# NonStopEagle137/Visual-Inertial-Odometry-MSCKF-Stereo

Measured on AMD Instinct MI355X. Metric: EKF measurement updates/sec at 30 cam-states x 200 features; ATE RMSE vs ref, higher is better.
Workload: dtype f32/f64; 1 GPU; batched EKF measurement update, 30 cam-states x 200 features, 2048 filters/GPU, triangulation + jacobian + gating + information assembly + Kalman, no row cap; cam_states=30, features=200, filters_per_gpu=2048, parallelism=replicas1

## Files before the change

visual-inertial-odometry-msckf-stereo_amd/csrc/msckf_kalman.hip:

```cpp
#include "msckf_common.h"
#include "msckf_launch.h"
#include "msckf_mchol_slots.h"
#include "msckf_rchol.h"

#include <stdlib.h>
#include <type_traits>

namespace msckf {

constexpr int KW = 24;

__device__ __forceinline__ int round4(int x) { return (x + 3) & ~3; }


typedef double v4d __attribute__((ext_vector_type(4)));

constexpr double KALMAN_PIVOT_FLOOR = 1e-10;

template <typename T>
__device__ double diag_max(const T* M, int ld, int o, int n, double* lds) {
    double m = 0.0;
    for (int i = threadIdx.x; i < n; i += blockDim.x) m = fmax(m, (double)M[(size_t)(o + i) * (ld + 1)]);
    m = wave_max(m);
    if ((threadIdx.x & 63) == 0) lds[threadIdx.x >> 6] = m;
    __syncthreads();
    for (int w = 0; w < (int)(blockDim.x >> 6); ++w) m = fmax(m, lds[w]);
    __syncthreads();
    return m;
}
template <typename T>
__device__ double pcc_pivot_floor(const T* P, int ld, int C, double* lds) {
    return diag_max(P, ld, 21, C, lds) * KALMAN_PIVOT_FLOOR;
}
constexpr double T_FLOOR_NEG = 1e-9;

template <typename T, int NT, int TPL, bool RETRY = false>
__global__ void __launch_bounds__(NT) __attribute__((amdgpu_waves_per_eu(NT == 256 ? 2 : 1))) k_kal_a(DevState<T> st, UpdWs<T> ws) {
    extern __shared__ __attribute__((aligned(16))) unsigned char smem_raw[];
    const int b = blockIdx.x;
    if (RETRY && ws.afail[b] == 0) return;
    const int C = 6 * st.ncams[b], Cp = round4(C);
    const int nrow = (Cp + KW) / 4;
    const T* P = st.P + (size_t)b * st.Dmax * st.Dmax;
    const int ld = st.Dmax, Cpw = ws.Cp;
    KT* Lc = ws.Lc + (size_t)b * Cpw * Cpw;
    KT* Vi = ws.Vi + (size_t)b * KW * Cpw;
    KT* Sii = ws.Sii + (size_t)b * KW * KW;
    auto map = [&](int i) { return i < C ? 21 + i : (i < Cp ? -1 : (i < Cp + 21 ? i - Cp : -1)); };
    double shift = 0.0;
    auto load = [&](int i, int j) -> double {
        const int mi = map(i), mj = map(j);
        if (mi < 0 || mj < 0) return i == j ? 1.0 : 0.0;
        return (double)P[(size_t)mi * ld + mj] + (i == j && i < C ? shift : 0.0);
    };
    auto panel = [&](int r, int c0, double w0, double w1, double w2, double w3) {
        KT* dst = r < Cp ? Lc + (size_t)r * Cpw + c0 : Vi + (size_t)(r - Cp) * Cpw + c0;
        dst[0] = w0; dst[1] = w1; dst[2] = w2; dst[3] = w3;
    };
    auto trail = [&](int i, int j, double v) { Sii[(i - Cp) * KW + (j - Cp)] = v; };
    const double floor = pcc_pivot_floor(P, ld, C, reinterpret_cast<double*>(smem_raw));
    bool ok = false;
    for (int att = RETRY ? 1 : 0; att < (RETRY ? 3 : 1) && !ok; ++att) {
        if (att > 0) {
            shift = (att == 1 ? 1e-8 : 1e-6) * (floor / KALMAN_PIVOT_FLOOR);
            __syncthreads();
        }
        ok = rchol_core<NT, TPL>(nrow, nrow, Cp / 4, reinterpret_cast<double*>(smem_raw), load, panel, trail, floor);
    }
    if (threadIdx.x == 0) ws.afail[b] = ok ? 0 : 1;
}

template <typename T, int NT, int TPL>
__global__ void __launch_bounds__(NT) __attribute__((amdgpu_waves_per_eu(NT == 256 ? 2 : 1))) k_kal_c1(DevState<T> st, UpdWs<T> ws) {
    extern __shared__ __attribute__((aligned(16))) unsigned char smem_raw[];
    const int b = blockIdx.x;
    if (ws.info[4 * b] == 0) return;
    if (ws.afail[b]) {
        if (threadIdx.x == 0) ws.info[4 * b + 3] = -2;
        return;
    }
    const int C = 6 * st.ncams[b], Cp = round4(C), nTc = Cp / 4;
    const int ldt = ws.Cmax + 1;
    const KT* Tm = ws.Tm + (size_t)b * ws.Cmax * ldt;
    KT* L = ws.G + (size_t)b * ws.Cmax * ldt;
    const bool rev = ws.rev;
    auto load = [&](int i, int j) -> double {
        if (i >= C || j >= C) return i == j ? 1.0 : 0.0;
        const int ri = rev ? C - 1 - i : i, rj = rev ? C - 1 - j : j;
        return ri >= rj ? Tm[(size_t)ri * ldt + rj] : Tm[(size_t)rj * ldt + ri];
    };
    auto panel = [&](int r, int c0, double w0, double w1, double w2, double w3) {
        if (r >= C) return;
        KT* dst = L + (size_t)r * ldt;
        const double w[4] = {w0, w1, w2, w3};
#pragma unroll
        for (int q = 0; q < 4; ++q)
            if (c0 + q < C && c0 + q <= r) dst[c0 + q] = w[q];
    };
    auto trail = [](int, int, double) {};
    const double tmax = diag_max(Tm, ldt, 0, C, reinterpret_cast<double*>(smem_raw));
    const bool ok = rchol_core<NT, TPL>(nTc, nTc, nTc, reinterpret_cast<double*>(smem_raw), load, panel, trail, ws.s2,
                                        -T_FLOOR_NEG * tmax);
    if (!ok && threadIdx.x == 0) ws.info[4 * b + 3] = -1;
}

constexpr int C2S = 17;

template <typename T, int NW, int CT, int NTM>
__global__ void __launch_bounds__(64 * NW) k_kal_c2(DevState<T> st, UpdWs<T> ws) {
    extern __shared__ __attribute__((aligned(16))) unsigned char smem_raw[];
    constexpr int NT = 64 * NW;
    const int b = blockIdx.x;
    if (ws.info[4 * b] == 0 || ws.info[4 * b + 3] < 0) return;
    const int C = 6 * st.ncams[b], nT = (C + 15) / 16, E = 22 + C, nE = (E + 15) / 16;
    const int tid = threadIdx.x, lane = tid & 63, lc = lane & 15, lr = lane >> 4;
    const int wv = __builtin_amdgcn_readfirstlane(tid >> 6);
    const int ldt = ws.Cmax + 1, Cpw = ws.Cp, ldw = st.Dmax + 1;
    const KT* L = ws.G + (size_t)b * ws.Cmax * ldt;
    const KT* Tm = ws.Tm + (size_t)b * ws.Cmax * ldt;
    const KT* Lc = ws.Lc + (size_t)b * Cpw * Cpw;
    const KT* Vi = ws.Vi + (size_t)b * KW * Cpw;
    KT* Wt = ws.W + (size_t)b * (st.Dmax + 1) * Cpw;
    double* LI = reinterpret_cast<double*>(smem_raw);
    double* img = LI + NTM * 256;
    auto Lv = [&](int r, int k) -> double {
        if (r >= C || k >= C) return r == k ? 1.0 : 0.0;
        return k <= r ? L[(size_t)r * ldt + k] : 0.0;
    };
    for (int J = wv; J < nT; J += NW) {
        double* blk = img + wv * 272;
#pragma unroll
        for (int q = 0; q < 4; ++q) {
            const int e = lane + 64 * q, i = e >> 4, k = e & 15;
            blk[e] = Lv(16 * J + i, 16 * J + k);
        }
        __builtin_amdgcn_wave_barrier();
        __builtin_amdgcn_fence(__ATOMIC_ACQ_REL, "wavefront");
        if (lane < 16) blk[256 + lane] = 1.0 / blk[17 * lane];
        __builtin_amdgcn_wave_barrier();
        __builtin_amdgcn_fence(__ATOMIC_ACQ_REL, "wavefront");
        if (lane < 16) {
            double x[16];
#pragma unroll
            for (int i = 0; i < 16; ++i) {
                double sv = i == lane ? 1.0 : 0.0;
#pragma unroll
                for (int k = 0; k < i; ++k) sv -= k >= lane ? blk[16 * i + k] * x[k] : 0.0;
                x[i] = i < lane ? 0.0 : sv * blk[256 + i];
            }
            double* xj = LI + J * 256 + 16 * lane;
#pragma unroll
            for (int i = 0; i < 16; ++i) xj[i] = x[i];
        }
        __builtin_amdgcn_wave_barrier();
        __builtin_amdgcn_fence(__ATOMIC_ACQ_REL, "wavefront");
    }
    const bool rev = ws.rev;
    auto Xv = [&](int e, int k) -> double {
        if (k >= C) return 0.0;
        const int j = rev ? C - 1 - k : k;
        if (e < 21) return Vi[(size_t)e * Cpw + j];
        if (e < 21 + C) return j <= e - 21 ? Lc[(size_t)(e - 21) * Cpw + j] : 0.0;
        if (e == 21 + C) return Tm[(size_t)j * ldt + C];
        return 0.0;
    };
    v4d yk[CT][NTM];
    int J0[CT];
#pragma unroll
// ... 265 lines not shown
#pragma unroll
        for (int q = 0; q < NLD; ++q) {
            int ii, kk, jj, k2;
            idx(q, A_KFAST, ii, kk);
            idx(q, B_KFAST, jj, k2);
            const int gi = i0 + ii, gk = k0 + kk;
            ra[q] = (gi < m && gk < ke) ? A(gi, gk) : 0.0;
            const int gj = j0 + jj, gk2 = k0 + k2;
            rb[q] = (gj < n && gk2 < ke) ? B(gk2, gj) : 0.0;
        }
    };
    auto sstore = [&](int bf) {
#pragma unroll
        for (int q = 0; q < NLD; ++q) {
            int ii, kk, jj, k2;
            idx(q, A_KFAST, ii, kk);
            idx(q, B_KFAST, jj, k2);
            sa[bf][kk][ii] = ra[q];
            sb[bf][k2][jj] = rb[q];
        }
    };
    if (kb < ke) {
        gload(kb);
        sstore(0);
    }
    __syncthreads();
    for (int k0 = kb, it = 0; k0 < ke; k0 += GK, ++it) {
        const int bf = it & 1;
        const bool more = k0 + GK < ke;
        if (more) gload(k0 + GK);
#pragma unroll
        for (int kc = 0; kc < GK / 4; ++kc) {
            const int kr = 4 * kc + lr;
            double av[NBW], bv[NBW];
#pragma unroll
            for (int t = 0; t < NBW; ++t) {
                av[t] = sa[bf][kr][HW * wr + 16 * t + lc];
                bv[t] = sb[bf][kr][HW * wc + 16 * t + lc];
            }
#pragma unroll
            for (int mi = 0; mi < NBW; ++mi)
#pragma unroll
                for (int ni = 0; ni < NBW; ++ni)
                    acc[mi][ni] = __builtin_amdgcn_mfma_f64_16x16x4f64(av[mi], bv[ni], acc[mi][ni], 0, 0, 0);
        }
        if (more) sstore(bf ^ 1);
        __syncthreads();
    }
#pragma unroll
    for (int mi = 0; mi < NBW; ++mi)
#pragma unroll
        for (int ni = 0; ni < NBW; ++ni)
#pragma unroll
            for (int r = 0; r < 4; ++r) {
                const int i = i0 + HW * wr + 16 * mi + lr + 4 * r, j = j0 + HW * wc + 16 * ni + lc;
                if (i < m && j < n) store(i, j, acc[mi][ni][r]);
            }
}
template <bool A_KFAST, bool B_KFAST, class FA, class FB, class FS>
__device__ __forceinline__ void gemm64(int m, int n, int kb, int ke, int i0, int j0, FA A, FB B, FS store) {
    gemm_tile<64, A_KFAST, B_KFAST>(m, n, kb, ke, i0, j0, A, B, store);
}

template <int STAGE, typename T>
__global__ void __launch_bounds__(256) k_gchol_trsm(DevState<T> st, UpdWs<T> ws, int k) {
    const Blk3 bk = xcd_blk3();
    const int b = bk.y;
    KT* A;
    int nrow, ncol, nelim;
    if (!gdims<STAGE>(st, ws, b, A, nrow, ncol, nelim) || k >= nelim) return;
    const int ld = ncol, nb = nelim - k < GNB ? nelim - k : GNB;
    const int i0 = k + nb + bk.x * GT;
    if (i0 >= nrow) return;
    const KT* Li = ws.G + (size_t)b * ws.Cmax * (ws.Cmax + 1);
    gemm64<true, true>(nrow, nb, 0, nb, i0, 0,
                       [&](int i, int p) { return A[(size_t)i * ld + k + p]; },
                       [&](int p, int j) { return Li[j * GNB + p]; },
                       [&](int i, int j, double v) { A[(size_t)i * ld + k + j] = v; });
}

template <int STAGE, typename T>
__global__ void __launch_bounds__(256) k_gchol_update(DevState<T> st, UpdWs<T> ws, int k) {
    const Blk3 bk = xcd_blk3();
    const int b = bk.z;
    KT* A;
    int nrow, ncol, nelim;
    if (!gdims<STAGE>(st, ws, b, A, nrow, ncol, nelim) || k >= nelim) return;
    const int ld = ncol, k1 = k + (nelim - k < GNB ? nelim - k : GNB);
    const int i0 = k1 + bk.y * GT, j0 = k1 + bk.x * GT;
    if (i0 >= nrow || j0 >= ncol || i0 + GT - 1 < j0) return;
    gemm64<true, true>(nrow, ncol, k, k1, i0, j0,
                       [&](int i, int p) { return A[(size_t)i * ld + p]; },
                       [&](int p, int j) { return A[(size_t)j * ld + p]; },
                       [&](int i, int j, double v) {
                           if (j <= i) A[(size_t)i * ld + j] -= v;
                       });
}

template <typename T>
__global__ void __launch_bounds__(256) k_kal_b1(DevState<T> st, UpdWs<T> ws) {
    const Blk3 bk = xcd_blk3();
    const int b = bk.z;
    if (ws.info[4 * b] == 0) return;
    const int C = 6 * st.ncams[b];
    const int i0 = bk.y * GT, j0 = bk.x * GT;
    if (i0 >= C || j0 >= C) return;
    const int lda = ws.Cmax + 1, Cpw = ws.Cp;
    const KT* Am = ws.Hthin + (size_t)b * ws.Cmax * lda;
    const KT* Lc = ws.Lc + (size_t)b * Cpw * Cpw;
    KT* G = ws.G + (size_t)b * ws.Cmax * lda;
    gemm64<true, false>(C, C, j0 & ~(GK - 1), C, i0, j0,
                        [&](int i, int k) { return Am[(size_t)i * lda + k]; },
                        [&](int k, int j) { return k >= j ? Lc[(size_t)k * Cpw + j] : 0.0; },
                        [&](int i, int j, double v) { G[(size_t)i * lda + j] = v; });
}

template <typename T>
__global__ void __launch_bounds__(256) k_kal_b2(DevState<T> st, Params<T> prm, UpdWs<T> ws) {
    const Blk3 bk = xcd_blk3();
    const int b = bk.z;
    if (ws.info[4 * b] == 0) return;
    const int C = 6 * st.ncams[b];
    const int i0 = bk.y * GT, j0 = bk.x * GT;
    if (i0 >= C || j0 > C) return;
    if (j0 > i0 + GT - 1 && !(C >= j0 && C < j0 + GT)) return;
    const int ld = ws.Cmax + 1, Cpw = ws.Cp;
    const KT* Lc = ws.Lc + (size_t)b * Cpw * Cpw;
    const KT* G = ws.G + (size_t)b * ws.Cmax * ld;
    const KT* Hb = ws.Hthin + (size_t)b * ws.Cmax * ld;
    KT* Tm = ws.Tm + (size_t)b * ws.Cmax * ld;
    KT* Ac = ws.Wk + (size_t)b * ws.wk_stride + gchol_c_off(ws.Cmax);
    const double s2 = (double)prm.sigma2;
    gemm64<false, false>(C, C + 1, i0 & ~(GK - 1), C, i0, j0,
                         [&](int i, int k) { return k >= i ? Lc[(size_t)k * Cpw + i] : 0.0; },
                         [&](int k, int j) { return j < C ? G[(size_t)k * ld + j] : Hb[(size_t)k * ld + ws.Cmax]; },
                         [&](int i, int j, double v) {
                             if (j < C && j <= i) {
                                 const double t = v + (i == j ? s2 : 0.0);
                                 Ac[(size_t)i * C + j] = t;
                                 if (i == j) Tm[(size_t)i * ld + i] = t;
                             }
                             if (j == C) Ac[(size_t)(2 * C + 21) * C + i] = v;
                         });
}

__device__ __forceinline__ void lower_tile(int t, int& ti, int& tj) {
    int i = (int)((sqrtf(8.0f * (float)t + 1.0f) - 1.0f) * 0.5f);
    while (i * (i + 1) / 2 > t) --i;
    while ((i + 1) * (i + 2) / 2 <= t) ++i;
    ti = i;
    tj = t - i * (i + 1) / 2;
}

template <typename T, int NW, int NTM>
__global__ void __launch_bounds__(64 * NW) k_kal_b(DevState<T> st, Params<T> prm, UpdWs<T> ws) {
    constexpr int TP2 = (NTM * (NTM + 1) / 2 + NW - 1) / NW;
    constexpr int NT = 64 * NW, Q = (16 * 16 * NTM + NT - 1) / NT;
    extern __shared__ __attribute__((aligned(16))) unsigned char smem_raw[];
    const int b = blockIdx.x;
    if (ws.info[4 * b] == 0) return;
    const int C = 6 * st.ncams[b], nT = (C + 15) / 16, Cq = 16 * nT;
    const int tid = threadIdx.x, lane = tid & 63, lc = lane & 15, lr = lane >> 4;
    const int wv = __builtin_amdgcn_readfirstlane(tid >> 6);
    const int ld = ws.Cmax + 1, Cpw = ws.Cp;
    const KT* Am = ws.Hthin + (size_t)b * ws.Cmax * ld;
    const KT* Lc = ws.Lc + (size_t)b * Cpw * Cpw;
    KT* G = ws.G + (size_t)b * ws.Cmax * ld;
    KT* Tm = ws.Tm + (size_t)b * ws.Cmax * ld;
    const int CqS1 = (Cq & ~31) + 17, CqS2 = (Cq & ~31) + 16;
    double* img = reinterpret_cast<double*>(smem_raw);
    double* bb = img + 4 * 16 * CqS1;
    double r0[Q], r1[Q], rb = 0.0;
    int pos[Q];
    auto load = [&](int ph, int k0) {
#pragma unroll
        for (int q = 0; q < Q; ++q) {
            const int e = tid + NT * q;
            int k, c;
            if (ph == 0) {
                const int jt = e >> 8, u = e & 255;
                const bool up = jt > (k0 >> 4);
                k = up ? (u & 15) : (u >> 4);
                c = 16 * jt + (up ? (u >> 4) : (u & 15));
            } else {
                k = e / Cq;
                c = e - k * Cq;
            }
            const int gk = k0 + k;
            pos[q] = k * (ph == 0 ? CqS1 : CqS2) + c;
            const bool in = e < 16 * Cq && gk < C && c < C;
            const double lcv = (in && c <= gk) ? Lc[(size_t)gk * Cpw + c] : 0.0;
            double ov;
            if (ph == 0) {
                ov = in ? Am[c <= gk ? (size_t)gk * ld + c : (size_t)c * ld + gk] : 0.0;
            } else {
                ov = (in && c < 16 * (gk / 16 + 1)) ? G[(size_t)gk * ld + c] : 0.0;
            }
            r0[q] = ph == 0 ? ov : lcv;
            r1[q] = ph == 0 ? lcv : ov;
        }
        if (ph == 1 && tid < 16) rb = k0 + tid < C ? Am[(size_t)(k0 + tid) * ld + ws.Cmax] : 0.0;
    };
    auto put = [&](int ph, int buf) {
        const int CqS = ph == 0 ? CqS1 : CqS2;
        double* i0 = img + (2 * buf) * 16 * CqS;
#pragma unroll
        for (int q = 0; q < Q; ++q) {
            const int e = tid + NT * q;
            if (e < 16 * Cq) {
                i0[pos[q]] = r0[q];
                i0[16 * CqS + pos[q]] = r1[q];
            }
        }
        if (ph == 1 && tid < 16) bb[buf * 16 + tid] = rb;
    };
    {
        const int CqS = CqS1;
        const int ntl = nT * (nT + 1) / 2;
        v4d acc[TP2];
        int gr[TP2], gc[TP2];
#pragma unroll
        for (int s = 0; s < TP2; ++s) {
            const int t = wv + NW * s, tt = t < ntl ? t : 0;
            const int c = colmajor_col(tt, nT), r = c + tt - (c * nT - c * (c - 1) / 2);
            gr[s] = __builtin_amdgcn_readfirstlane(t < ntl ? r : -1);
            gc[s] = __builtin_amdgcn_readfirstlane(c);
            acc[s] = v4d{0.0, 0.0, 0.0, 0.0};
        }
        load(0, 0);
        put(0, 0);
        __syncthreads();
        for (int k0 = 0, it = 0; k0 < C; k0 += 16, ++it) {
            const int buf = it & 1;
            const bool more = k0 + 16 < C;
            if (more) load(0, k0 + 16);
            const double* i0 = img + (2 * buf) * 16 * CqS;
            const double* i1 = i0 + 16 * CqS;
#pragma unroll
            for (int kc = 0; kc < 4; ++kc) {
                const int kr = (4 * kc + lr) * CqS;
#pragma unroll
                for (int s = 0; s < TP2; ++s) {
                    if (gr[s] < 0 || k0 + 15 < 16 * gc[s]) continue;
                    acc[s] = __builtin_amdgcn_mfma_f64_16x16x4f64(i0[kr + 16 * gr[s] + lc], i1[kr + 16 * gc[s] + lc],
                                                                  acc[s], 0, 0, 0);
                }
            }
            if (more) put(0, buf ^ 1);
            __syncthreads();
        }
#pragma unroll
        for (int s = 0; s < TP2; ++s) {
            if (gr[s] < 0) continue;
#pragma unroll
            for (int r = 0; r < 4; ++r) {
                const int i = 16 * gr[s] + lr + 4 * r, j = 16 * gc[s] + lc;
                if (i < C && j < C) G[(size_t)i * ld + j] = acc[s][r];
            }
        }
        __syncthreads();
    }
    {
        const int CqS = CqS2;
        const int ntl = nT * (nT + 1) / 2;
        v4d acc[TP2];
        int ti[TP2], tj[TP2];
#pragma unroll
        for (int s = 0; s < TP2; ++s) {
            const int t = wv + NW * s;
            int x, y;
            lower_tile(t, x, y);
            ti[s] = __builtin_amdgcn_readfirstlane(t < ntl ? x : -1);
            tj[s] = __builtin_amdgcn_readfirstlane(y);
            acc[s] = v4d{0.0, 0.0, 0.0, 0.0};
        }
        double ca = 0.0;
        load(1, 0);
        put(1, 0);
        __syncthreads();
        for (int k0 = 0, it = 0; k0 < C; k0 += 16, ++it) {
            const int buf = it & 1;
            const bool more = k0 + 16 < C;
            if (more) load(1, k0 + 16);
            const double* i0 = img + (2 * buf) * 16 * CqS;
            const double* i1 = i0 + 16 * CqS;
#pragma unroll
            for (int kc = 0; kc < 4; ++kc) {
                const int kr = (4 * kc + lr) * CqS;
#pragma unroll
                for (int s = 0; s < TP2; ++s) {
                    if (ti[s] < 0 || k0 + 15 < 16 * ti[s]) continue;
                    acc[s] = __builtin_amdgcn_mfma_f64_16x16x4f64(i0[kr + 16 * ti[s] + lc], i1[kr + 16 * tj[s] + lc],
                                                                  acc[s], 0, 0, 0);
                }
            }
            if (tid < C) {
#pragma unroll
                for (int k = 0; k < 16; ++k) ca += i0[k * CqS + tid] * bb[buf * 16 + k];
            }
            if (more) put(1, buf ^ 1);
            __syncthreads();
        }
        const double s2 = (double)prm.sigma2;
#pragma unroll
        for (int s = 0; s < TP2; ++s) {
            if (ti[s] < 0) continue;
#pragma unroll
            for (int r = 0; r < 4; ++r) {
                const int i = 16 * ti[s] + lr + 4 * r, j = 16 * tj[s] + lc;
                if (i < C && j <= i) Tm[(size_t)i * ld + j] = acc[s][r] + (i == j ? s2 : 0.0);
            }
        }
        if (tid < C) Tm[(size_t)tid * ld + C] = ca;
    }
}

template <typename T>
__global__ void __launch_bounds__(256) __attribute__((amdgpu_waves_per_eu(2))) k_kal_e(DevState<T> st, Params<T> prm, UpdWs<T> ws) {
    constexpr int TE = 128;
    const Blk3 bk = xcd_blk3();
    const int b = bk.z;
    if (ws.info[4 * b] == 0 || ws.info[4 * b + 3] < 0) return;
    const int C = 6 * st.ncams[b], D = 21 + C;
    const int i0 = bk.y * TE, j0 = bk.x * TE;
    if (i0 >= D || j0 > D) return;
    if (j0 > i0 + TE - 1 && !(D >= j0 && D < j0 + TE)) return;
    const int ld = st.Dmax;
    const KT* W = ws.Wk + (size_t)b * ws.wk_stride + gchol_c_off(ws.Cmax) + (size_t)C * C;
    const KT* Sii = ws.Sii + (size_t)b * KW * KW;
    T* P = st.P + (size_t)b * st.Dmax * st.Dmax;
    KT* dx = ws.dx + (size_t)b * (st.Dmax + ws.Cmax);
    const double s2 = (double)prm.sigma2;
    gemm_tile<TE, true, true>(D, D + 1, 0, C, i0, j0, [&](int i, int k) { return W[(size_t)i * C + k]; },
                       [&](int k, int j) { return W[(size_t)(j < D ? j : D) * C + k]; },
                       [&](int i, int j, double v) {
                           if (j < D && j <= i) {
                               double p = s2 * v;
                               if (i < 21 && j < 21) p += Sii[i * KW + j];
                               P[(size_t)i * ld + j] = (T)p;
                               P[(size_t)j * ld + i] = (T)p;
                           }
                           if (j == D) dx[i] = v;
                       });
}

template <typename T, int NW, int TPW>
__global__ void __launch_bounds__(64 * NW) k_kal_e1(DevState<T> st, Params<T> prm, UpdWs<T> ws) {
    extern __shared__ __attribute__((aligned(16))) unsigned char smem_raw[];
    const int b = blockIdx.x;
    if (ws.info[4 * b] == 0 || ws.info[4 * b + 3] < 0) return;
    const int C = 6 * st.ncams[b], D = 21 + C, nT = (D + 15) / 16, Dp = 16 * nT;
    const int tid = threadIdx.x, lane = tid & 63, lc = lane & 15, lr = lane >> 4;
    const int wv = __builtin_amdgcn_readfirstlane(tid >> 6);
    const int ntiles = nT * (nT + 1) / 2;
    const int Cpw = ws.Cp, ld = st.Dmax;
    const KT* W = ws.W + (size_t)b * (st.Dmax + 1) * Cpw;
    double* img = reinterpret_cast<double*>(smem_raw);
    double* yb = img + 2 * 16 * Dp;
    int ti[TPW], tj[TPW], kf[TPW];
#pragma unroll
    for (int s = 0; s < TPW; ++s) {
        const int t = wv + NW * s;
        int c = 0, rem = t;
        if (rem >= nT) {
            rem -= nT;
            c = 1;
            if (rem >= nT - 1) {
                rem -= nT - 1;
                c = nT - 1;
                while (c > 1 && rem >= nT - c) { rem -= nT - c; --c; }
            }
        }
        const int rmax = (16 * c + 15 < D ? 16 * c + 15 : D - 1) - 21;
        ti[s] = __builtin_amdgcn_readfirstlane(t < ntiles ? c + rem : -1);
        tj[s] = __builtin_amdgcn_readfirstlane(c);
        kf[s] = __builtin_amdgcn_readfirstlane(ws.rev && c >= 2 ? (C - 1 - rmax) / 16 : 0);
    }
    v4d acc[TPW];
#pragma unroll
    for (int s = 0; s < TPW; ++s) acc[s] = v4d{0.0, 0.0, 0.0, 0.0};
    double dxa = 0.0, dxb = 0.0;
    constexpr int NT = 64 * NW, Q = (16 * 16 * (NW * TPW <= 96 ? 13 : 15) + NT - 1) / NT;
    double rw[Q], ry = 0.0;
    const int ldw = st.Dmax + 1;
    auto load = [&](int k0) {
#pragma unroll
        for (int q = 0; q < Q; ++q) {
            const int e = tid + NT * q;
            const int k = e / Dp, row = e - k * Dp, gk = k0 + k;
            const bool zero = ws.rev && row >= 21 && gk + row - 21 < C - 1;
            rw[q] = (e < 16 * Dp && row < D && gk < C && !zero) ? W[(size_t)gk * ldw + row] : 0.0;
        }
        if (tid < 16) ry = k0 + tid < C ? W[(size_t)(k0 + tid) * ldw + D] : 0.0;
    };
    auto put = [&](int buf) {
        double* im = img + buf * 16 * Dp;
#pragma unroll
        for (int q = 0; q < Q; ++q) {
            const int e = tid + NT * q;
            if (e < 16 * Dp) im[e] = rw[q];
        }
        if (tid < 16) yb[buf * 16 + tid] = ry;
    };
    load(0);
    put(0);
    __syncthreads();
    for (int k0 = 0, it = 0; k0 < C; k0 += 16, ++it) {
        const int buf = it & 1;
        const bool more = k0 + 16 < C;
        if (more) load(k0 + 16);
        const double* im = img + buf * 16 * Dp;
#pragma unroll
        for (int kc = 0; kc < 4; ++kc) {
            const double* kr = im + (4 * kc + lr) * Dp;
#pragma unroll
            for (int s = 0; s < TPW; ++s) {
                if (ti[s] < 0 || it < kf[s]) continue;
                acc[s] = __builtin_amdgcn_mfma_f64_16x16x4f64(kr[16 * ti[s] + lc], kr[16 * tj[s] + lc], acc[s], 0, 0, 0);
            }
        }
        if (tid < D) {
#pragma unroll
            for (int k = 0; k < 16; ++k) dxa += im[k * Dp + tid] * yb[buf * 16 + k];
        }
        if (NT + tid < D) {
#pragma unroll
            for (int k = 0; k < 16; ++k) dxb += im[k * Dp + NT + tid] * yb[buf * 16 + k];
        }
        if (more) put(buf ^ 1);
        __syncthreads();
    }
    const double s2 = (double)prm.sigma2;
    const KT* Sii = ws.Sii + (size_t)b * KW * KW;
    T* P = st.P + (size_t)b * st.Dmax * st.Dmax;
#pragma unroll
    for (int s = 0; s < TPW; ++s) {
        if (ti[s] < 0) continue;
#pragma unroll
        for (int r = 0; r < 4; ++r) {
            const int i = 16 * ti[s] + lr + 4 * r, j = 16 * tj[s] + lc;
            if (i >= D || j >= D || j > i) continue;
            double p = s2 * acc[s][r];
            if (i < 21 && j < 21) p += Sii[i * KW + j];
            P[(size_t)i * ld + j] = (T)p;
            P[(size_t)j * ld + i] = (T)p;
        }
    }
    if (tid < D) ws.dx[(size_t)b * (st.Dmax + ws.Cmax) + tid] = dxa;
    if (NT + tid < D) ws.dx[(size_t)b * (st.Dmax + ws.Cmax) + NT + tid] = dxb;
}

constexpr int MK_PS = 4;
__host__ __device__ constexpr int mk_lookahead(int SL) { return SL > 20 ? 1 : 2; }

__device__ __forceinline__ double mk_rcp(double x) {
    const double r = __builtin_amdgcn_rcp(x);
    return r * fma(-x, r, 2.0);
}

__host__ __device__ constexpr int mk_lds_doubles(int NBR) { return 2 * 16 * NBR * MK_PS + 16; }

template <int N, class Fn>
__device__ __forceinline__ void mk_static_for(Fn&& f) {
    if constexpr (N > 0) {
        mk_static_for<N - 1>(f);
        f(std::integral_constant<int, N - 1>{});
    }
}

template <typename T, int NW, int NBR, int WV>
__device__ __forceinline__ bool mk_wave(const DevState<T>& st, const UpdWs<T>& ws, int b, double floor, double lo,
                                        double* pan0) {
    constexpr int SL = mk_nslots(NBR, NW), JN = mk_used_slots(NBR, NW, WV), MK_LA = mk_lookahead(SL);
    const int tid = threadIdx.x, lane = tid & 63, lc = lane & 15, lr = lane >> 4;
    const int C = 6 * st.ncams[b], Cp = round4(C);
    const int nrows = C;
    const int nsteps = Cp / 4;
    const int ldt = ws.Cmax + 1;
    const KT* Tm = ws.Tm + (size_t)b * ws.Cmax * ldt;
    KT* LT = ws.G + (size_t)b * ws.Cmax * ldt;
    auto load = [&](int i, int j) -> double {
        const bool pad = i >= C || j >= C;
        const int ri = ws.rev ? C - 1 - i : i, rj = ws.rev ? C - 1 - j : j;
        const double v = Tm[pad ? (size_t)0 : (ri >= rj ? (size_t)ri * ldt + rj : (size_t)rj * ldt + ri)];
        return pad ? (i == j ? 1.0 : 0.0) : v;
    };
    using v4d_t = double __attribute__((ext_vector_type(4)));
    v4d_t acc[SL];
    mk_static_for<JN>([&](auto jc) {
        constexpr int j = decltype(jc)::value, r = mk_brow(NBR, NW, WV, j), c = mk_bcol(NBR, NW, WV, j);
#pragma unroll
        for (int q = 0; q < 4; ++q) acc[j][q] = load(16 * r + lr + 4 * q, 16 * c + lc);
        __builtin_amdgcn_sched_barrier(0);
    });
    const double oh[4] = {lr == 0 ? 1.0 : 0.0, lr == 1 ? 1.0 : 0.0, lr == 2 ? 1.0 : 0.0, lr == 3 ? 1.0 : 0.0};
    int status = 0;
    mk_static_for<NBR>([&](auto kbc) {
      constexpr int KB = decltype(kbc)::value;
      constexpr int J0 = mk_first_slot(NBR, NW, WV, KB), J1 = mk_first_slot(NBR, NW, WV, KB + 1);
      if (status != 0) return;
#pragma nounroll
      for (int sc = 0; sc < 4; ++sc) {
        if (4 * KB + sc >= nsteps) { status = 1; break; }
        const int p0 = 16 * KB + 4 * sc;
        double* pan = pan0 + (sc & 1) * 16 * NBR * MK_PS;
        if ((lc >> 2) == sc) {
            double* d = pan + lr * MK_PS + (lc & 3);
            mk_static_for<J1 - J0>([&](auto jc) {
                constexpr int j = J0 + decltype(jc)::value, r = mk_brow(NBR, NW, WV, j);
#pragma unroll
                for (int q = 0; q < 4; ++q) d[(16 * r + 4 * q) * MK_PS] = acc[j][q];
            });
        }
        __syncthreads();
        const double* ad = pan + p0 * MK_PS;
        const double a10 = ad[4], a20 = ad[8], a30 = ad[12];
        const double a21 = ad[9], a31 = ad[13], a32 = ad[14];
        const double d0 = pivot_floored(ad[0], floor, lo), e0 = mk_rcp(d0);
        const double l10 = a10 * e0, l20 = a20 * e0, l30 = a30 * e0;
        const double d1 = pivot_floored(ad[5] - l10 * a10, floor, lo), e1 = mk_rcp(d1);
        const double m21 = a21 - l20 * a10, m31 = a31 - l30 * a10;
        const double l21 = m21 * e1, l31 = m31 * e1;
        const double d2 = pivot_floored(ad[10] - l20 * a20 - l21 * m21, floor, lo), e2 = mk_rcp(d2);
        const double m32 = a32 - l30 * a20 - l31 * m21;
        const double l32 = m32 * e2;
        const double d3 = pivot_floored(ad[15] - l30 * a30 - l31 * m31 - l32 * m32, floor, lo), e3 = mk_rcp(d3);
        if (__builtin_amdgcn_readfirstlane((int)(!(d0 > 0.0) || !(d1 > 0.0) || !(d2 > 0.0) || !(d3 > 0.0)))) {
            status = 2;
            break;
        }
        {
            const int r = p0 + tid;
            if (r < nrows) {
                const double* x = pan + r * MK_PS;
                const double z0 = x[0], z1 = x[1] - l10 * z0, z2 = x[2] - l20 * z0 - l21 * z1;
                const double z3 = x[3] - l30 * z0 - l31 * z1 - l32 * z2;
                const int k = r - p0;
                const double y0 = (k == 0 ? d0 : z0) * rchol_rsq(d0);
                const double y1 = k >= 1 ? (k == 1 ? d1 : z1) * rchol_rsq(d1) : 0.0;
                const double y2 = k >= 2 ? (k == 2 ? d2 : z2) * rchol_rsq(d2) : 0.0;
                const double y3 = k >= 3 ? (k == 3 ? d3 : z3) * rchol_rsq(d3) : 0.0;
                KT* dst = LT + (size_t)r * ldt + p0;
                dst[0] = y0;
                if (p0 + 1 < C) dst[1] = y1;
                if (p0 + 2 < C) dst[2] = y2;
                if (p0 + 3 < C) dst[3] = y3;
            }
        }
        const double h0 = oh[0];
        const double h1 = fma(-l10, h0, oh[1]);
        const double h2 = fma(-l21, h1, fma(-l20, h0, oh[2]));
        const double h3 = fma(-l32, h2, fma(-l31, h1, fma(-l30, h0, oh[3])));
        const double u0 = h0 * e0, u1 = h1 * e1, u2 = h2 * e2, u3 = h3 * e3;
        const double w2 = fma(-l32, u3, u2);
        const double w1 = fma(-l31, u3, fma(-l21, w2, u1));
        const double w0 = fma(-l30, u3, fma(-l20, w2, fma(-l10, w1, u0)));
        const double* pa = pan + lc * MK_PS;
        const double* pb = pan + lc * MK_PS + lr;
        double x[SL][4], bv[NBR];
        auto update = [&](auto jac, auto jbc) {
            constexpr int JA = decltype(jac)::value, JB = decltype(jbc)::value;
            auto ldo = [&](auto jc) {
                constexpr int j = decltype(jc)::value;
                if constexpr (j < JB) {
                    constexpr int r = mk_brow(NBR, NW, WV, j), c = mk_bcol(NBR, NW, WV, j);
#pragma unroll
                    for (int i = 0; i < 4; ++i) x[j][i] = pa[16 * r * MK_PS + i];
                    if constexpr (j == JA || mk_bcol(NBR, NW, WV, j - 1) != c) bv[c] = pb[16 * c * MK_PS];
                }
            };
            mk_static_for<MK_LA>([&](auto lc_) { ldo(std::integral_constant<int, JA + decltype(lc_)::value>{}); });
            mk_static_for<JB - JA>([&](auto jc) {
                constexpr int j = JA + decltype(jc)::value, c = mk_bcol(NBR, NW, WV, j);
                ldo(std::integral_constant<int, j + MK_LA>{});
                const double av = -fma(x[j][3], u3, fma(x[j][2], w2, fma(x[j][0], w0, x[j][1] * w1)));
                acc[j] = __builtin_amdgcn_mfma_f64_16x16x4f64(av, bv[c], acc[j], 0, 0, 0);
            });
        };
        __builtin_amdgcn_sched_barrier(0);
        if constexpr (J1 > J0)
            if (sc < 3) update(std::integral_constant<int, J0>{}, std::integral_constant<int, J1>{});
        update(std::integral_constant<int, J1>{}, std::integral_constant<int, JN>{});
      }
    });
    return status != 2;
}

template <typename T, int NW, int NBR, int STAGE>
__device__ __forceinline__ bool mk_factor(const DevState<T>& st, const UpdWs<T>& ws, int b, double shift,
                                          double floor, double lo, double* pan0) {
    if constexpr (STAGE == 1) {
        static_assert(NW == 4, "one mk_wave code path per wave");
        bool ok = false;
        switch (__builtin_amdgcn_readfirstlane(threadIdx.x >> 6)) {
        case 0: ok = mk_wave<T, NW, NBR, 0>(st, ws, b, floor, lo, pan0); break;
        case 1: ok = mk_wave<T, NW, NBR, 1>(st, ws, b, floor, lo, pan0); break;
        case 2: ok = mk_wave<T, NW, NBR, 2>(st, ws, b, floor, lo, pan0); break;
        default: ok = mk_wave<T, NW, NBR, 3>(st, ws, b, floor, lo, pan0); break;
        }
        __syncthreads();
        return ok;
    }
    constexpr int NBLK = NBR * (NBR + 1) / 2, SL = (NBLK + NW - 1) / NW;
    const int tid = threadIdx.x, lane = tid & 63, lc = lane & 15, lr = lane >> 4;
    const int wv = __builtin_amdgcn_readfirstlane(tid >> 6);
    const int C = 6 * st.ncams[b], Cp = round4(C);
    const int nrows = STAGE == 0 ? Cp + KW : C;
    const int nsteps = Cp / 4;
    const int ld = st.Dmax, Cpw = ws.Cp, ldt = ws.Cmax + 1;
    const T* P = st.P + (size_t)b * st.Dmax * st.Dmax;
    KT* Lc = ws.Lc + (size_t)b * Cpw * Cpw;
    KT* Vi = ws.Vi + (size_t)b * KW * Cpw;
    KT* Sii = ws.Sii + (size_t)b * KW * KW;
    const KT* Tm = ws.Tm + (size_t)b * ws.Cmax * ldt;
    KT* LT = ws.G + (size_t)b * ws.Cmax * ldt;
    auto map = [&](int i) { return i < C ? 21 + i : (i < Cp ? -1 : (i < Cp + 21 ? i - Cp : -1)); };
    auto load = [&](int i, int j) -> double {
        if (STAGE == 0) {
            const int mi = map(i), mj = map(j);
            if (mi < 0 || mj < 0) return i == j ? 1.0 : 0.0;
            return (double)P[(size_t)mi * ld + mj] + (i == j && i < C ? shift : 0.0);
// ... 356 lines not shown
```

Before: 301,100 updates/s.

## Add compile-time tile maps for full-size Kalman GEMM kernels

Adds specialized code paths for the information-assembly (k_kal_b) and covariance-update (k_kal_e1) kernels when the tile count matches a fixed size. A constexpr header assigns lower-triangular 16x16 tiles to waves statically. Triangular skipping is resolved as a runtime count over compile-time ordered slots, and MFMA operands are batched in pairs. This is meant to remove runtime tile-index computation and let accumulators stay in registers with unrolled addressing. The cost is more code size and register pressure, and the path only applies to one specific problem size.

```diff
diff --git a/visual-inertial-odometry-msckf-stereo_amd/csrc/msckf_kalman.hip b/visual-inertial-odometry-msckf-stereo_amd/csrc/msckf_kalman.hip
--- a/visual-inertial-odometry-msckf-stereo_amd/csrc/msckf_kalman.hip
+++ b/visual-inertial-odometry-msckf-stereo_amd/csrc/msckf_kalman.hip
@@ -1,5 +1,6 @@
 #include "msckf_common.h"
 #include "msckf_launch.h"
+#include "msckf_kalman_tiles.h"
 #include "msckf_mchol_slots.h"
 #include "msckf_rchol.h"
 
@@ -14,6 +15,14 @@
 
 
 typedef double v4d __attribute__((ext_vector_type(4)));
+
+template <int N, class Fn>
+__device__ __forceinline__ void mk_static_for(Fn&& f) {
+    if constexpr (N > 0) {
+        mk_static_for<N - 1>(f);
+        f(std::integral_constant<int, N - 1>{});
+    }
+}
 
 constexpr double KALMAN_PIVOT_FLOOR = 1e-10;
 
@@ -585,6 +594,184 @@
     tj = t - i * (i + 1) / 2;
 }
 
+
+template <int DEAL, int NTM, int NW, int WV>
+__device__ __forceinline__ int kt_count(int it, int q) {
+    int n = 0;
+    mk_static_for<kt_used(DEAL, NTM, NW, WV)>([&](auto sc) {
+        constexpr int s = decltype(sc)::value;
+        constexpr int key = kt_key(DEAL, kt_row(DEAL, NTM, NW, WV, s), kt_col(DEAL, NTM, NW, WV, s));
+        if constexpr (key == KT_ALWAYS) ++n;
+        else n += (DEAL == KT_E ? it + key >= q : it >= key) ? 1 : 0;
+    });
+    return n;
+}
+
+constexpr int KT_BATCH = 2;
+template <int DEAL, int NTM, int NW, int WV, int STRIDE>
+__device__ __forceinline__ void kt_mfma(int it, int q, const double* p0, const double* p1, v4d* acc) {
+    const int n = kt_count<DEAL, NTM, NW, WV>(it, q);
+    mk_static_for<kt_used(DEAL, NTM, NW, WV)>([&](auto sc) {
+        constexpr int s = decltype(sc)::value;
+        constexpr int R = kt_row(DEAL, NTM, NW, WV, s), Cc = kt_col(DEAL, NTM, NW, WV, s);
+        if (s >= n) return;
+#pragma unroll
+        for (int h = 0; h < 4; h += KT_BATCH) {
+            double x[KT_BATCH], y[KT_BATCH];
+#pragma unroll
+            for (int kc = 0; kc < KT_BATCH; ++kc) {
+                x[kc] = p0[4 * (h + kc) * STRIDE + 16 * R];
+                y[kc] = p1[4 * (h + kc) * STRIDE + 16 * Cc];
+            }
+#pragma unroll
+            for (int kc = 0; kc < KT_BATCH; ++kc)
+                acc[s] = __builtin_amdgcn_mfma_f64_16x16x4f64(x[kc], y[kc], acc[s], 0, 0, 0);
+        }
+    });
+}
+
+template <int NW, class Fn>
+__device__ __forceinline__ void kt_per_wave(int wv, Fn&& f) {
+    mk_static_for<NW>([&](auto wc) {
+        if (wv == decltype(wc)::value) f(wc);
+    });
+}
+
+__host__ __device__ constexpr bool kb_has_map(int NW, int NTM) { return NW == 16 && NTM == 12; }
+
+template <typename T, int NW, int NTM>
+__device__ __forceinline__ void kb_full(const DevState<T>& st, const Params<T>& prm, const UpdWs<T>& ws, int b, int wv,
+                                        unsigned char* smem_raw) {
+    constexpr int SL = kt_nslots(NTM, NW);
+    constexpr int NT = 64 * NW, Q = (16 * 16 * NTM + NT - 1) / NT;
+    constexpr int Cq = 16 * NTM, CqS1 = (Cq & ~31) + 17, CqS2 = (Cq & ~31) + 16;
+    const int C = 6 * st.ncams[b];
+    const int tid = threadIdx.x, lane = tid & 63, lc = lane & 15, lr = lane >> 4;
+    const int ld = ws.Cmax + 1, Cpw = ws.Cp;
+    const KT* Am = ws.Hthin + (size_t)b * ws.Cmax * ld;
+    const KT* Lc = ws.Lc + (size_t)b * Cpw * Cpw;
+    KT* G = ws.G + (size_t)b * ws.Cmax * ld;
+    KT* Tm = ws.Tm + (size_t)b * ws.Cmax * ld;
+    double* img = reinterpret_cast<double*>(smem_raw);
+    double* bb = img + 4 * 16 * CqS1;
+    double r0[Q], r1[Q], rb = 0.0;
+    int pos[Q];
+    auto load = [&](int ph, int k0) {
+#pragma unroll
+        for (int q = 0; q < Q; ++q) {
+            const int e = tid + NT * q;
+            int k, c;
+            if (ph == 0) {
+                const int jt = e >> 8, u = e & 255;
+                const bool up = jt > (k0 >> 4);
+                k = up ? (u & 15) : (u >> 4);
+                c = 16 * jt + (up ? (u >> 4) : (u & 15));
+            } else {
+                k = e / Cq;
+                c = e - k * Cq;
+            }
+            const int gk = k0 + k;
+            pos[q] = k * (ph == 0 ? CqS1 : CqS2) + c;
+            const bool in = e < 16 * Cq && gk < C && c < C;
+            const double lcv = (in && c <= gk) ? Lc[(size_t)gk * Cpw + c] : 0.0;
+            double ov;
+            if (ph == 0) {
+                ov = in ? Am[c <= gk ? (size_t)gk * ld + c : (size_t)c * ld + gk] : 0.0;
+            } else {
+                ov = (in && c < 16 * (gk / 16 + 1)) ? G[(size_t)gk * ld + c] : 0.0;
+            }
+            r0[q] = ph == 0 ? ov : lcv;
+            r1[q] = ph == 0 ? lcv : ov;
+        }
+        if (ph == 1 && tid < 16) rb = k0 + tid < C ? Am[(size_t)(k0 + tid) * ld + ws.Cmax] : 0.0;
+    };
+    auto put = [&](int ph, int buf) {
+        const int CqS = ph == 0 ? CqS1 : CqS2;
+        double* i0 = img + (2 * buf) * 16 * CqS;
+#pragma unroll
+        for (int q = 0; q < Q; ++q) {
+            const int e = tid + NT * q;
+            if (e < 16 * Cq) {
+                i0[pos[q]] = r0[q];
+                i0[16 * CqS + pos[q]] = r1[q];
+            }
+        }
+        if (ph == 1 && tid < 16) bb[buf * 16 + tid] = rb;
+    };
+    {
+        constexpr int CqS = CqS1;
+        v4d acc[SL];
+#pragma unroll
+        for (int s = 0; s < SL; ++s) acc[s] = v4d{0.0, 0.0, 0.0, 0.0};
+        load(0, 0);
+        put(0, 0);
+        __syncthreads();
+        for (int k0 = 0, it = 0; k0 < C; k0 += 16, ++it) {
+            const int buf = it & 1;
+            const bool more = k0 + 16 < C;
+            if (more) load(0, k0 + 16);
+            const double* i0 = img + (2 * buf) * 16 * CqS + lr * CqS + lc;
+            kt_per_wave<NW>(wv, [&](auto wc) {
+                kt_mfma<KT_B1, NTM, NW, decltype(wc)::value, CqS>(it, 0, i0, i0 + 16 * CqS, acc);
+            });
+            if (more) put(0, buf ^ 1);
+            __syncthreads();
+        }
+        kt_per_wave<NW>(wv, [&](auto wc) {
+            constexpr int WV = decltype(wc)::value;
+            mk_static_for<kt_used(KT_B1, NTM, NW, WV)>([&](auto sc) {
+                constexpr int s = decltype(sc)::value;
+                constexpr int gr = kt_row(KT_B1, NTM, NW, WV, s), gc = kt_col(KT_B1, NTM, NW, WV, s);
+#pragma unroll
+                for (int r = 0; r < 4; ++r) {
+                    const int i = 16 * gr + lr + 4 * r, j = 16 * gc + lc;
+                    if (i < C && j < C) G[(size_t)i * ld + j] = acc[s][r];
+                }
+            });
+        });
+        __syncthreads();
+    }
+    {
+        constexpr int CqS = CqS2;
+        v4d acc[SL];
+#pragma unroll
+        for (int s = 0; s < SL; ++s) acc[s] = v4d{0.0, 0.0, 0.0, 0.0};
+        double ca = 0.0;
+        load(1, 0);
+        put(1, 0);
+        __syncthreads();
+        for (int k0 = 0, it = 0; k0 < C; k0 += 16, ++it) {
+            const int buf = it & 1;
+            const bool more = k0 + 16 < C;
+            if (more) load(1, k0 + 16);
+            const double* i0 = img + (2 * buf) * 16 * CqS;
+            kt_per_wave<NW>(wv, [&](auto wc) {
+                kt_mfma<KT_B2, NTM, NW, decltype(wc)::value, CqS>(it, 0, i0 + lr * CqS + lc, i0 + (16 + lr) * CqS + lc, acc);
+            });
+            if (tid < C) {
+#pragma unroll
+                for (int k = 0; k < 16; ++k) ca += i0[k * CqS + tid] * bb[buf * 16 + k];
+            }
+            if (more) put(1, buf ^ 1);
+            __syncthreads();
+        }
+        const double s2 = (double)prm.sigma2;
+        kt_per_wave<NW>(wv, [&](auto wc) {
+            constexpr int WV = decltype(wc)::value;
+            mk_static_for<kt_used(KT_B2, NTM, NW, WV)>([&](auto sc) {
+                constexpr int s = decltype(sc)::value;
+                constexpr int ti = kt_row(KT_B2, NTM, NW, WV, s), tj = kt_col(KT_B2, NTM, NW, WV, s);
+#pragma unroll
+                for (int r = 0; r < 4; ++r) {
+                    const int i = 16 * ti + lr + 4 * r, j = 16 * tj + lc;
+                    if (i < C && j <= i) Tm[(size_t)i * ld + j] = acc[s][r] + (i == j ? s2 : 0.0);
+                }
+            });
+        });
+        if (tid < C) Tm[(size_t)tid * ld + C] = ca;
+    }
+}
+
 template <typename T, int NW, int NTM>
 __global__ void __launch_bounds__(64 * NW) k_kal_b(DevState<T> st, Params<T> prm, UpdWs<T> ws) {
     constexpr int TP2 = (NTM * (NTM + 1) / 2 + NW - 1) / NW;
@@ -595,6 +782,12 @@
     const int C = 6 * st.ncams[b], nT = (C + 15) / 16, Cq = 16 * nT;
     const int tid = threadIdx.x, lane = tid & 63, lc = lane & 15, lr = lane >> 4;
     const int wv = __builtin_amdgcn_readfirstlane(tid >> 6);
+    if constexpr (kb_has_map(NW, NTM)) {
+        if (nT == NTM) {
+            kb_full<T, NW, NTM>(st, prm, ws, b, wv, smem_raw);
+            return;
+        }
+    }
     const int ld = ws.Cmax + 1, Cpw = ws.Cp;
     const KT* Am = ws.Hthin + (size_t)b * ws.Cmax * ld;
     const KT* Lc = ws.Lc + (size_t)b * Cpw * Cpw;
@@ -777,6 +970,90 @@
                        });
 }
 
+__host__ __device__ constexpr int e1_ntm(int NW, int TPW) { return NW * TPW <= 96 ? 13 : 15; }
+#ifndef MSCKF_KT_E1
+#define MSCKF_KT_E1 1
+#endif
+__host__ __device__ constexpr bool e1_has_map(int NW, int TPW) { return MSCKF_KT_E1 && NW == 16 && TPW == 6; }
+
+template <typename T, int NW, int TPW>
+__device__ __forceinline__ void e1_full(const DevState<T>& st, const Params<T>& prm, const UpdWs<T>& ws, int b, int wv,
+                                        unsigned char* smem_raw) {
+    constexpr int NTM = e1_ntm(NW, TPW), SL = kt_nslots(NTM, NW), Dp = 16 * NTM;
+    static_assert(kt_nslots(NTM, NW) <= TPW, "accumulator slots");
+    const int C = 6 * st.ncams[b], D = 21 + C;
+    const int tid = threadIdx.x, lane = tid & 63, lc = lane & 15, lr = lane >> 4;
+    const int Cpw = ws.Cp, ld = st.Dmax;
+    const KT* W = ws.W + (size_t)b * (st.Dmax + 1) * Cpw;
+    double* img = reinterpret_cast<double*>(smem_raw);
+    double* yb = img + 2 * 16 * Dp;
+    const int qf = ws.rev ? (C + 5) >> 4 : 0;
+    v4d acc[SL];
+#pragma unroll
+    for (int s = 0; s < SL; ++s) acc[s] = v4d{0.0, 0.0, 0.0, 0.0};
+    double dxa = 0.0;
+    constexpr int NT = 64 * NW, Q = (16 * 16 * NTM + NT - 1) / NT;
+    static_assert(NT >= Dp, "one dx row per thread");
+    double rw[Q], ry = 0.0;
+    const int ldw = st.Dmax + 1;
+    auto load = [&](int k0) {
+#pragma unroll
+        for (int q = 0; q < Q; ++q) {
+            const int e = tid + NT * q;
+            const int k = e / Dp, row = e - k * Dp, gk = k0 + k;
+            const bool zero = ws.rev && row >= 21 && gk + row - 21 < C - 1;
+            rw[q] = (e < 16 * Dp && row < D && gk < C && !zero) ? W[(size_t)gk * ldw + row] : 0.0;
+        }
+        if (tid < 16) ry = k0 + tid < C ? W[(size_t)(k0 + tid) * ldw + D] : 0.0;
+    };
+    auto put = [&](int buf) {
+        double* im = img + buf * 16 * Dp;
+#pragma unroll
+        for (int q = 0; q < Q; ++q) {
+            const int e = tid + NT * q;
+            if (e < 16 * Dp) im[e] = rw[q];
+        }
+        if (tid < 16) yb[buf * 16 + tid] = ry;
+    };
+    load(0);
+    put(0);
+    __syncthreads();
+    for (int k0 = 0, it = 0; k0 < C; k0 += 16, ++it) {
+        const int buf = it & 1;
+        const bool more = k0 + 16 < C;
+        if (more) load(k0 + 16);
+        const double* im = img + buf * 16 * Dp;
+        const double* kr = im + lr * Dp + lc;
+        kt_per_wave<NW>(wv, [&](auto wc) { kt_mfma<KT_E, NTM, NW, decltype(wc)::value, Dp>(it, qf, kr, kr, acc); });
+        if (tid < D) {
+#pragma unroll
+            for (int k = 0; k < 16; ++k) dxa += im[k * Dp + tid] * yb[buf * 16 + k];
+        }
+        if (more) put(buf ^ 1);
+        __syncthreads();
+    }
+    const double s2 = (double)prm.sigma2;
+    const KT* Sii = ws.Sii + (size_t)b * KW * KW;
+    T* P = st.P + (size_t)b * st.Dmax * st.Dmax;
+    kt_per_wave<NW>(wv, [&](auto wc) {
+        constexpr int WV = decltype(wc)::value;
+        mk_static_for<kt_used(KT_E, NTM, NW, WV)>([&](auto sc) {
+            constexpr int s = decltype(sc)::value;
+            constexpr int ti = kt_row(KT_E, NTM, NW, WV, s), tj = kt_col(KT_E, NTM, NW, WV, s);
+#pragma unroll
+            for (int r = 0; r < 4; ++r) {
+                const int i = 16 * ti + lr + 4 * r, j = 16 * tj + lc;
+                if (i >= D || j >= D || j > i) continue;
+                double p = s2 * acc[s][r];
+                if (i < 21 && j < 21) p += Sii[i * KW + j];
+                P[(size_t)i * ld + j] = (T)p;
+                P[(size_t)j * ld + i] = (T)p;
+            }
+        });
+    });
+    if (tid < D) ws.dx[(size_t)b * (st.Dmax + ws.Cmax) + tid] = dxa;
+}
+
 template <typename T, int NW, int TPW>
 __global__ void __launch_bounds__(64 * NW) k_kal_e1(DevState<T> st, Params<T> prm, UpdWs<T> ws) {
     extern __shared__ __attribute__((aligned(16))) unsigned char smem_raw[];
@@ -785,6 +1062,12 @@
     const int C = 6 * st.ncams[b], D = 21 + C, nT = (D + 15) / 16, Dp = 16 * nT;
     const int tid = threadIdx.x, lane = tid & 63, lc = lane & 15, lr = lane >> 4;
     const int wv = __builtin_amdgcn_readfirstlane(tid >> 6);
+    if constexpr (e1_has_map(NW, TPW)) {
+        if (nT == e1_ntm(NW, TPW)) {
+            e1_full<T, NW, TPW>(st, prm, ws, b, wv, smem_raw);
+            return;
+        }
+    }
     const int ntiles = nT * (nT + 1) / 2;
     const int Cpw = ws.Cp, ld = st.Dmax;
     const KT* W = ws.W + (size_t)b * (st.Dmax + 1) * Cpw;
@@ -892,14 +1175,6 @@
 }
 
 __host__ __device__ constexpr int mk_lds_doubles(int NBR) { return 2 * 16 * NBR * MK_PS + 16; }
-
-template <int N, class Fn>
-__device__ __forceinline__ void mk_static_for(Fn&& f) {
-    if constexpr (N > 0) {
-        mk_static_for<N - 1>(f);
-        f(std::integral_constant<int, N - 1>{});
-    }
-}
 
 template <typename T, int NW, int NBR, int WV>
 __device__ __forceinline__ bool mk_wave(const DevState<T>& st, const UpdWs<T>& ws, int b, double floor, double lo,
diff --git a/visual-inertial-odometry-msckf-stereo_amd/csrc/msckf_kalman_tiles.h b/visual-inertial-odometry-msckf-stereo_amd/csrc/msckf_kalman_tiles.h
--- /dev/null
+++ b/visual-inertial-odometry-msckf-stereo_amd/csrc/msckf_kalman_tiles.h
@@ -0,0 +1,102 @@
+#pragma once
+
+namespace msckf {
+
+enum { KT_B1 = 0, KT_B2 = 1, KT_E = 2 };
+
+constexpr int kt_ntiles(int NTM) { return NTM * (NTM + 1) / 2; }
+constexpr int kt_nslots(int NTM, int NW) { return (kt_ntiles(NTM) + NW - 1) / NW; }
+
+constexpr int kt_col_of(int DEAL, int NTM, int t) {
+    if (DEAL == KT_B2) {
+        int r = 0, rem = t;
+        while (rem > r) { rem -= r + 1; ++r; }
+        return rem;
+    }
+    int n = 0, rem = t;
+    for (;; ++n) {
+        const int c = DEAL == KT_B1 ? n : (n < 2 ? n : NTM + 1 - n);
+        if (rem < NTM - c) return c;
+        rem -= NTM - c;
+    }
+}
+constexpr int kt_row_of(int DEAL, int NTM, int t) {
+    if (DEAL == KT_B2) {
+        int r = 0, rem = t;
+        while (rem > r) { rem -= r + 1; ++r; }
+        return r;
+    }
+    int n = 0, rem = t;
+    for (;; ++n) {
+        const int c = DEAL == KT_B1 ? n : (n < 2 ? n : NTM + 1 - n);
+        if (rem < NTM - c) return c + rem;
+        rem -= NTM - c;
+    }
+}
+
+constexpr int kt_row(int DEAL, int NTM, int NW, int WV, int s) {
+    return WV + NW * s < kt_ntiles(NTM) ? kt_row_of(DEAL, NTM, WV + NW * s) : -1;
+}
+constexpr int kt_col(int DEAL, int NTM, int NW, int WV, int s) {
+    return WV + NW * s < kt_ntiles(NTM) ? kt_col_of(DEAL, NTM, WV + NW * s) : -1;
+}
+constexpr int kt_used(int DEAL, int NTM, int NW, int WV) {
+    int n = 0;
+    while (n < kt_nslots(NTM, NW) && WV + NW * n < kt_ntiles(NTM)) ++n;
+    return n;
+}
+
+constexpr int KT_ALWAYS = 1 << 20;
+constexpr int kt_key(int DEAL, int r, int c) {
+    return DEAL == KT_B1 ? c : DEAL == KT_B2 ? r : (c < 2 ? KT_ALWAYS : c);
+}
+constexpr bool kt_reached(int DEAL, int r, int c, int it, int q) {
+    return DEAL == KT_E ? it + kt_key(DEAL, r, c) >= q : it >= kt_key(DEAL, r, c);
+}
+constexpr int kt_nact(int DEAL, int NTM, int NW, int WV, int it, int q) {
+    int n = 0;
+    for (int s = 0; s < kt_used(DEAL, NTM, NW, WV); ++s)
+        if (kt_reached(DEAL, kt_row(DEAL, NTM, NW, WV, s), kt_col(DEAL, NTM, NW, WV, s), it, q)) ++n;
+    return n;
+}
+constexpr bool kt_count_occurs(int DEAL, int NTM, int NW, int WV, int n) {
+    const int u = kt_used(DEAL, NTM, NW, WV);
+    if (n < 1 || n > u) return false;
+    if (n == u) return true;
+    return kt_key(DEAL, kt_row(DEAL, NTM, NW, WV, n - 1), kt_col(DEAL, NTM, NW, WV, n - 1)) !=
+           kt_key(DEAL, kt_row(DEAL, NTM, NW, WV, n), kt_col(DEAL, NTM, NW, WV, n));
+}
+
+constexpr bool kt_map_ok(int DEAL, int NTM, int NW) {
+    if (NTM > 16) return false;
+    int owners[16 * 16] = {};
+    for (int w = 0; w < NW; ++w) {
+        int used = 0;
+        for (int s = 0; s < kt_nslots(NTM, NW); ++s) {
+            const int r = kt_row(DEAL, NTM, NW, w, s), c = kt_col(DEAL, NTM, NW, w, s);
+            if (r < 0) continue;
+            if (c < 0 || c > r || r >= NTM || used != s) return false;
+            ++owners[16 * r + c];
+            ++used;
+        }
+        if (used != kt_used(DEAL, NTM, NW, w)) return false;
+    }
+    for (int c = 0; c < NTM; ++c)
+        for (int r = c; r < NTM; ++r)
+            if (owners[16 * r + c] != 1) return false;
+    for (int t = 1; t < kt_ntiles(NTM); ++t) {
+        const int k0 = kt_key(DEAL, kt_row_of(DEAL, NTM, t - 1), kt_col_of(DEAL, NTM, t - 1));
+        const int k1 = kt_key(DEAL, kt_row_of(DEAL, NTM, t), kt_col_of(DEAL, NTM, t));
+        if (DEAL == KT_E ? k1 > k0 : k1 < k0) return false;
+    }
+    return true;
+}
+
+static_assert(kt_map_ok(KT_B1, 8, 8) && kt_map_ok(KT_B2, 8, 8), "k_kal_b<8, 8> tile maps");
+static_assert(kt_map_ok(KT_B1, 12, 16) && kt_map_ok(KT_B2, 12, 16), "k_kal_b<16, 12> tile maps");
+static_assert(kt_map_ok(KT_E, 13, 16), "k_kal_e1<16, 6> tile map");
+static_assert(kt_map_ok(KT_E, 15, 8), "k_kal_e1<8, 16> tile map");
+static_assert(kt_nslots(12, 16) == 5 && kt_nslots(8, 8) == 5 && kt_nslots(13, 16) == 6 && kt_nslots(15, 8) == 15,
+              "accumulators per wave");
+
+}
```

Measured after the change: 285,700 updates/s. 0.949x the previous value.
